# ViacheslavTimofeev/tpu_superresolution

Measured on AMD Instinct MI355X. Metric: HR pixels/sec, SwinIR x4 train step, 64x64 LR, bs=32/GPU, higher is better.
Workload: dtype bf16; 1 GPU; BASELINE cfg3: SwinIR classical x4 (dim 180, 6x6 blocks, window 8) train step = fwd + L1 + bwd + clip 1.0 + AdamW, 64x64 LR patches -> 256x256 HR, random-init weights, drop_path 0.1; every step starts from the seeded weights and fresh AdamW state; batch_per_gpu=32, global_batch=32, parallelism=dp1

## Files before the change

tpu_superresolution_amd/csrc/api.hip:

```cpp
#include <stdarg.h>
#include <stdio.h>
#include <string.h>

#include "adamw.h"
#include "kernels.h"
#include "wgrad.h"

static thread_local char g_err[512] = "";

SrkOptTls& srk_opt_tls() {
  static thread_local SrkOptTls t = {};
  return t;
}

static SrkOpt** opt_table() {
  static SrkOpt* table[SRK_NUM_OPTS] = {};
  return table;
}

void srk_opt_register(SrkOpt* o) {
  if (o->id >= 0 && o->id < SRK_NUM_OPTS) opt_table()[o->id] = o;
}

void srk_opt_scope_begin(SrkOptTls* saved) {
// ... 323 lines not shown
  srk_wgrad_stream_tune_get(&rows, &nt);
  return which == 0 ? rows : nt;
}

struct OptEntry {
  const char* name;
  int (*get)();
  int (*set)(int);
};

const OptEntry kOptions[] = {
    {"gemm_stream", [] { return srk_gemm_stream_enabled(); }, [](int v) { srk_gemm_stream_enable(v); return (int)SRK_OK; }},
    {"attn_bwd_fused", [] { return srk_attn_bwd_fused_enabled(); }, [](int v) { srk_attn_bwd_fused_enable(v); return (int)SRK_OK; }},
    {"attn_fused", [] { return srk_attn_fused_mode(); }, [](int v) { srk_attn_fused_enable(v); return (int)SRK_OK; }},
    {"wgrad_stream_w8", [] { return srk_wgrad_w8_enabled(); }, [](int v) { srk_wgrad_w8_enable(v); return (int)SRK_OK; }},
    {"block_light", [] { return srk_block_light_enabled(); }, [](int v) { srk_block_light_enable(v); return (int)SRK_OK; }},
    {"mlp_bwd_fused", [] { return srk_mlp_bwd_fused_enabled(); }, [](int v) { srk_mlp_bwd_fused_enable(v); return (int)SRK_OK; }},
    {"mlp_dgelu_store", [] { return srk_mlp_dgelu_store_enabled(); }, [](int v) { srk_mlp_dgelu_store_enable(v); return (int)SRK_OK; }},
    {"mlp_fused", [] { return srk_mlp_fused_enabled(); }, [](int v) { srk_mlp_fused_enable(v); return (int)SRK_OK; }},
    {"wgrad_stream", [] { return srk_wgrad_stream_enabled(); }, [](int v) { srk_wgrad_stream_enable(v); return (int)SRK_OK; }},
    {"conv_wgrad_taps", [] { return srk_conv_wgrad_taps_mode(); }, [](int v) { srk_conv_wgrad_taps_enable(v); return (int)SRK_OK; }},
    {"conv_wgrad_roll", [] { return srk_conv_wgrad_roll_enabled(); }, [](int v) { srk_conv_wgrad_roll_enable(v); return (int)SRK_OK; }},
    {"wgrad_partials", [] { return srk_wgrad_partials_enabled(); }, [](int v) { srk_wgrad_partials_enable(v); return (int)SRK_OK; }},
    {"wgrad_stream_rows", [] { return wtune_get(0); },
     [](int v) {
       SRK_REQUIRE(v == 32 || v == 64, SRK_E_SHAPE, "wgrad_stream_rows: 32/64");
       srk_wgrad_stream_tune(v, -1);
       return (int)SRK_OK;
     }},
    {"wgrad_stream_nt", [] { return wtune_get(1); }, [](int v) { srk_wgrad_stream_tune(0, v != 0); return (int)SRK_OK; }},
    {"gemm_stream_bm", [] { return tune_get(0); },
     [](int v) {
       SRK_REQUIRE(v == 0 || v == 16 || v == 32 || v == 64, SRK_E_SHAPE, "gemm_stream_bm: 0/16/32/64");
       return tune_set(0, v);
     }},
    {"gemm_stream_ks2", [] { return tune_get(1); }, [](int v) { return tune_set(1, v < 0 ? -1 : (v != 0)); }},
    {"gemm_stream_split", [] { return tune_get(2); }, [](int v) { return tune_set(2, v < 0 ? -1 : (v != 0)); }},
    {"gemm_stream_nb", [] { return tune_get(3); },
     [](int v) {
       SRK_REQUIRE(v == 0 || v == 4 || v == 8, SRK_E_SHAPE, "gemm_stream_nb: 0/4/8");
       return tune_set(3, v);
     }},
    {"probe_stride", [] { return g_probe.stride; },
     [](int v) {
       SRK_REQUIRE(v >= 1 && v <= 1024, SRK_E_SHAPE, "probe_stride: 1..1024");
       g_probe.stride = v;
// ... 246 lines not shown
```

tpu_superresolution_amd/csrc/common.h:

```cpp
#pragma once
#include <hip/hip_runtime.h>
#include <stdint.h>

#include "../../include/srk.h"

typedef unsigned short bf16_t;
typedef __attribute__((ext_vector_type(8))) short bf16x8_t;
typedef __attribute__((ext_vector_type(4))) short bf16x4_t;
typedef __attribute__((ext_vector_type(4))) float f32x4_t;

#define SRK_WAVE 64

void srk_set_error(const char* fmt, ...);
int srk_check_launch(const char* what);

constexpr int SRK_MAX_DEVICES = 64;
int srk_current_device();
int srk_device_cus();
enum SrkOptId {
  OPT_MLP_FUSED, OPT_MLP_BWD_FUSED, OPT_GEMM_STREAM, OPT_TUNE_BM, OPT_TUNE_KS2, OPT_TUNE_SPLIT, OPT_TUNE_NB, OPT_ATTN_BWD_FUSED,
  OPT_ATTN_FUSED, OPT_BLOCK_LIGHT, OPT_TAPS_ENABLED, OPT_TAPS_DMA, OPT_WGRAD_STREAM, OPT_WGRAD_ROWS, OPT_WGRAD_NT, OPT_WGRAD_W8,
  OPT_WGRAD_PARTIALS, OPT_MLP_DGELU_STORE, OPT_TAPS_ROLL, SRK_NUM_OPTS
};
struct SrkOptTls {
  int v[SRK_NUM_OPTS];
  unsigned on;
};
SrkOptTls& srk_opt_tls();
struct SrkOpt;
void srk_opt_register(SrkOpt* o);
void srk_opt_scope_begin(SrkOptTls* saved);
void srk_opt_scope_end(const SrkOptTls& saved);
struct SrkOpt {
  int id;
  int value;
  SrkOpt(int id_, int v) : id(id_), value(v) { srk_opt_register(this); }
  operator int() const {
    const SrkOptTls& t = srk_opt_tls();
    return ((t.on >> id) & 1u) ? t.v[id] : value;
  }
  SrkOpt& operator=(int v) {
    SrkOptTls& t = srk_opt_tls();
    if ((t.on >> id) & 1u) t.v[id] = v;
    else value = v;
    return *this;
// ... 224 lines not shown
```

tpu_superresolution_amd/csrc/gemm.hip:

```cpp
#include "gemm.h"
#include "gemm_rowep.h"

namespace {

constexpr int BM = 128;
constexpr int BK = 64;

#ifndef SRK_GEMM_DMA
#define SRK_GEMM_DMA 1
#endif
__device__ uint4 g_gemm_zero[1];

template <int LD>
struct RowCtx {
  long long base[4];
  int yx[4];
};

template <int LD, int EP, int NT, bool NARROW>
__global__ __launch_bounds__(256) void gemm_kernel(const GemmParams p) {
  constexpr int BN = NARROW ? 16 : NT * 32;
  constexpr int WPASS = NARROW ? 1 : BN / 32;
  extern __shared__ __attribute__((aligned(16))) unsigned char smem[];
  bf16_t* As = reinterpret_cast<bf16_t*>(smem);
// ... 336 lines not shown
  SRK_REQUIRE(p.A && p.Wt, SRK_E_NULL, "gemm: null operand");
  if (loader != LD_ROWS) {
    SRK_REQUIRE(p.CinP % 64 == 0 && p.K == 9 * p.CinP && p.M == p.B * p.H * p.W, SRK_E_SHAPE,
                "conv: inconsistent geometry K=%d CinP=%d M=%d B*H*W=%d", p.K, p.CinP, p.M, p.B * p.H * p.W);
    SRK_REQUIRE(p.H < 32768 && p.W < 32768, SRK_E_SHAPE, "conv: image too large");
    if (loader == LD_CONV3_PS) SRK_REQUIRE(p.Cs % 64 == 0 && p.CinP == p.r * p.r * p.Cs, SRK_E_SHAPE, "conv(ps-in): bad Cs");
  } else {
    SRK_REQUIRE(p.lda >= p.K && p.lda % 8 == 0, SRK_E_SHAPE, "gemm: bad lda %d", p.lda);
  }
  if (p.xn_out) {
    SRK_REQUIRE((epilogue == EP_PROJ_RES || epilogue == EP_RES) && (p.N == 64 || p.N == 128 || p.N == 192), SRK_E_SHAPE,
                "gemm: fused LayerNorm output needs a residual epilogue and N in {64,128,192} (N=%d)", p.N);
    SRK_REQUIRE(p.xn_mean && p.xn_rstd && p.xn_gamma && p.xn_beta, SRK_E_NULL, "gemm: fused LayerNorm: null pointer");
  }
  if (epilogue == EP_LNBWD) {
    SRK_REQUIRE(loader == LD_ROWS && (p.N == 64 || p.N == 128 || p.N == 192), SRK_E_SHAPE, "gemm(ln-bwd epilogue): N=%d must be one tile (64/128/192)", p.N);
    SRK_REQUIRE(p.ln_x && p.ln_mean && p.ln_rstd && p.ln_gamma && p.ln_dgamma && p.ln_dbeta && p.outf, SRK_E_NULL,
                "gemm(ln-bwd epilogue): null pointer");
  }
  if (loader == LD_ROWS) {
    const int rc = srk_launch_gemm_stream(epilogue, p, stream);
    if (rc != SRK_NOT_COVERED) return rc;
  }
#define CASE(LD, EP) \
  if (loader == LD && epilogue == EP) return dispatch_nt<LD, EP>(p, stream);
  CASE(LD_ROWS, EP_BF16)
  CASE(LD_ROWS, EP_QKV)
  CASE(LD_ROWS, EP_PROJ_RES)
  CASE(LD_ROWS, EP_GELU)
  CASE(LD_ROWS, EP_RES)
  CASE(LD_ROWS, EP_DGELU)
  CASE(LD_ROWS, EP_LNBWD)
  CASE(LD_ROWS, EP_LRELU)
  CASE(LD_ROWS, EP_DLRELU)
  CASE(LD_CONV3, EP_RES)
  CASE(LD_CONV3, EP_RES_BF16)
  CASE(LD_CONV3, EP_LRELU)
  CASE(LD_CONV3, EP_PS)
  CASE(LD_CONV3, EP_BF16)
  CASE(LD_CONV3, EP_DLRELU)
  CASE(LD_CONV3, EP_F32_BF16)
  CASE(LD_CONV3, EP_GELU)
  CASE(LD_CONV3, EP_DGELU)
  CASE(LD_ROWS, EP_RES_BF16)
  CASE(LD_CONV3_PS, EP_BF16)
  CASE(LD_CONV3_PS, EP_DLRELU)
// ... 7 lines not shown
```

tpu_superresolution_amd/csrc/gemm_stream.hip:

```cpp
#include <hip/hip_runtime.h>

#include "gemm.h"
#include "gemm_rowep.h"

namespace {

constexpr int SBN = 192;
constexpr int SBNP = SBN + 4;
constexpr int NC = SBN / 64;
constexpr int LDS_BUDGET = 160 * 1024;

#ifndef SRK_NT_GEMM
#define SRK_NT_GEMM 1
#endif
#ifndef SRK_NT_STORE_U
#define SRK_NT_STORE_U 1
#endif
typedef unsigned srk_u2 __attribute__((ext_vector_type(2)));
typedef float srk_f4 __attribute__((ext_vector_type(4)));
#ifndef SRK_NT_STORE_ALL
#define SRK_NT_STORE_ALL 0
#endif
__device__ __forceinline__ void st_u2(bf16_t* ptr, uint2 v) {
  if constexpr (SRK_NT_STORE_ALL != 0) __builtin_nontemporal_store(srk_u2{v.x, v.y}, reinterpret_cast<srk_u2*>(ptr));
  else *reinterpret_cast<uint2*>(ptr) = v;
}
// ... 365 lines not shown
      for (int c = 0; c < NC; ++c) {
        const float4 old = *reinterpret_cast<const float4*>(e0 + C::E32_BYTES + lr * (SBN * 4) + (64 * c + 4 * j16) * 4);
        float o[4] = {old.x, old.y, old.z, old.w};
        if (p.ln_skip) {
          const float4 sk = *reinterpret_cast<const float4*>(p.ln_skip + t_ * p.ldo + 64 * c + 4 * j16);
          o[0] += sk.x; o[1] += sk.y; o[2] += sk.z; o[3] += sk.w;
        }
#pragma unroll
        for (int e = 0; e < 4; ++e) {
          if (64 * c + 4 * j16 + e < p.ln_C) {
            o[e] += rstd * (dy[c][e] * gm[c][e] - s1 - xh[c][e] * s2);
            cg[c][e] += dy[c][e] * xh[c][e];
            cb[c][e] += dy[c][e];
          }
        }
        st_f4(dst + t_ * p.ldo + 64 * c + 4 * j16, make_float4(o[0], o[1], o[2], o[3]));
        if (p.outb)
          st_u2(p.outb + ro * p.ldo + 64 * c + 4 * j16, pack_bf4(o[0] * f, o[1] * f, o[2] * f, o[3] * f));
      }
    }
  }
}

template <int EP, int KC, int BM, bool KS2>
__global__ __launch_bounds__(512) void gemm_stream_kernel(const GemmParams p, int nchunk, int groups_per_xcd) {
  using C = StreamCfg<EP, KC, BM>;
  constexpr int K = C::K, R = C::R, MF = BM / 16;
  constexpr int KST = KS2 ? K / 64 : K / 32;
  extern __shared__ __attribute__((aligned(16))) unsigned char smem[];
  float* T = reinterpret_cast<float*>(smem);
  float* colred = reinterpret_cast<float*>(smem + C::T_BYTES);
  const unsigned smem_base = (unsigned)(size_t)smem;
  constexpr int SLOTS_OFF = C::T_BYTES + C::RED_BYTES;

  const int tid = threadIdx.x, lane = tid & 63;
  const int wave = __builtin_amdgcn_readfirstlane(tid >> 6);
  const int r16 = lane & 15, g = lane >> 4;

  const int xcd = blockIdx.x & 7, sx = blockIdx.x >> 3;
  const int chunk = sx % nchunk, gx = sx / nchunk;
  if (gx >= groups_per_xcd) return;
  const int n0 = chunk * SBN;
  const int Gm = 8 * groups_per_xcd, gi = gx * 8 + xcd;
  const int ntm = p.M / BM;
  const int nt = gi < ntm ? (ntm - gi + Gm - 1) / Gm : 0;
  if (nt == 0) return;

  const bool mfma_wave = KS2 || wave < 4;
  const int wn = wave & 3, kh = KS2 ? (wave >> 2) : 0;

  bf16x8_t wf[3][KST];
  if (mfma_wave) {
#pragma unroll
    for (int j = 0; j < 3; ++j)
#pragma unroll
      for (int s = 0; s < KST; ++s)
        wf[j][s] = *reinterpret_cast<const bf16x8_t*>(p.Wt + (long long)(n0 + wn * 48 + 16 * j + r16) * K + (kh * KST + s) * 32 + g * 8);
#pragma unroll
    for (int j = 0; j < 3; ++j)
#pragma unroll
      for (int s = 0; s < KST; ++s) asm volatile("" ::"v"(wf[j][s]));
  }
  if constexpr (EP == EP_LNBWD) {
// ... 657 lines not shown
    *state = -1;
    return SRK_OK;
  }
  if (hipFuncSetAttribute(fn, hipFuncAttributeMaxDynamicSharedMemorySize, lds) != hipSuccess) {
    srk_set_error("gemm(stream): cannot reserve %d bytes of LDS", lds);
    return SRK_E_LAUNCH;
  }
  *state = 1;
  return SRK_OK;
}

template <int EP, int KC, int BM, int NB>
int launch_split(const GemmParams& p, hipStream_t stream) {
  using S = SplitCfg<EP, KC, BM>;
  if constexpr (!S::VALID || BM % (4 * NB) != 0 || (NB == 8 && (KC > 3 || EP == EP_LNBWD))) {
    return SRK_NOT_COVERED;
  } else {
    static SrkPerDevice<int> configured_pd; int& configured = configured_pd.here();
    const int rc = stream_configure(&gemm_stream_split_kernel<EP, KC, BM, NB>, S::LDS, &configured);
    if (rc) return rc;
    if (configured < 0) return SRK_NOT_COVERED;
    const int nchunk = p.N / SBN;
    const int per_xcd = g_num_cus / 8;
    srk_probe_pre(FAM_GEMM_LINEAR, stream, p.flops, p.bytes);
    hipLaunchKernelGGL((gemm_stream_split_kernel<EP, KC, BM, NB>), dim3(per_xcd * 8), dim3(64 * (NB + 4)), S::LDS, stream, p, nchunk, per_xcd / nchunk);
    srk_probe_post(FAM_GEMM_LINEAR, stream);
    return srk_check_launch("gemm(stream-split)");
  }
}

template <int EP, int KC, int BM, bool KS2>
int launch_stream(const GemmParams& p, hipStream_t stream) {
  using C = StreamCfg<EP, KC, BM>;
  if constexpr (!C::VALID || (KC == 9 && !KS2)) {
    return SRK_NOT_COVERED;
  } else {
    static SrkPerDevice<int> configured_pd; int& configured = configured_pd.here();
    const int rcc = stream_configure(&gemm_stream_kernel<EP, KC, BM, KS2>, C::LDS, &configured);
    if (rcc) return rcc;
    if (configured < 0) return SRK_NOT_COVERED;
    const int nchunk = p.N / SBN;
    const int per_xcd = g_num_cus / 8;
    const int groups_per_xcd = per_xcd / nchunk;
    srk_probe_pre(FAM_GEMM_LINEAR, stream, p.flops, p.bytes);
    hipLaunchKernelGGL((gemm_stream_kernel<EP, KC, BM, KS2>), dim3(per_xcd * 8), dim3(512), C::LDS, stream, p, nchunk, groups_per_xcd);
    srk_probe_post(FAM_GEMM_LINEAR, stream);
    return srk_check_launch("gemm(stream)");
  }
}

template <int EP, int KC>
int launch_cfg(const GemmParams& p, hipStream_t stream, int bm, bool ks2) {
  if (bm == 16) return ks2 ? launch_stream<EP, KC, 16, true>(p, stream) : launch_stream<EP, KC, 16, false>(p, stream);
  if (bm == 32) return ks2 ? launch_stream<EP, KC, 32, true>(p, stream) : launch_stream<EP, KC, 32, false>(p, stream);
  if (bm == 64) return ks2 ? launch_stream<EP, KC, 64, true>(p, stream) : launch_stream<EP, KC, 64, false>(p, stream);
  return SRK_NOT_COVERED;
}

template <int EP, int KC>
int launch_split_bm(const GemmParams& p, hipStream_t stream, int bm, int nb) {
  if (nb == 8) {
    if (bm == 32) return launch_split<EP, KC, 32, 8>(p, stream);
    if (bm == 64) return launch_split<EP, KC, 64, 8>(p, stream);
    return SRK_NOT_COVERED;
  }
  if (bm == 16) return launch_split<EP, KC, 16, 4>(p, stream);
  if (bm == 32) return launch_split<EP, KC, 32, 4>(p, stream);
  if (bm == 64) return launch_split<EP, KC, 64, 4>(p, stream);
// ... 137 lines not shown
```

tpu_superresolution_amd/csrc/swinir.hip:

```cpp
#include <string.h>

#include <map>
#include <string>
#include <vector>

#include "kernels.h"
#include "wgrad.h"

namespace {

struct ParamEntry {
  std::string name;
  long long off, numel;
  int ndim;
  long long shape[4];
};

struct BlockW {
  long long n1w, n1b, rpb, qkvw, qkvb, projw, projb, n2w, n2b, fc1w, fc1b, fc2w, fc2b;
  long long Wqkv, WqkvT, Wproj, WprojT, Wfc1, Wfc1T, Wfc2, Wfc2T;
  long long bqkv, bproj, bfc1, bfc2, biasd;
  int nH, dh, CA, shift;
  float scale;
};
// ... 1233 lines not shown
        wq[2] = lin_wgrad(c, c.at<bf16_t>(w.gxbw), CP, c.at<bf16_t>(ba.ao), bw.CA, T, bw.Wproj, bw.bproj, fl_proj);
        int nslab;
        if (w.attn_recompute) {
          const int rc_abf = srk_launch_qkv_attn_bwd(c.at<bf16_t>(ba.xn1w), CP, c.packed + bw.Wqkv, c.side + bw.bqkv, bw.scale,
                                                     c.at<bf16_t>(w.gxbw), CP, c.packed + bw.WprojT, c.side + bw.biasd,
                                                     c.at<bf16_t>(w.dqkv), c.at<float>(w.slab), T / 64, bw.nH, bw.CA, CP, geom, st);
          SRK_REQUIRE(rc_abf != SRK_NOT_COVERED, SRK_E_STATE, "backward: the re-projecting attention backward cannot run but the "
                      "forward stored no q/k/v (option attn_bwd_fused changed between forward and backward?)");
          RUN(rc_abf);
          nslab = srk_qkv_attn_bwd_slabs(T / 64, bw.nH, bw.CA, CP);
        } else {
          {
            GemmParams g = {};
            g.A = c.at<bf16_t>(w.gxbw); g.lda = CP; g.Wt = c.packed + bw.WprojT; g.M = T; g.N = bw.CA; g.K = CP;
            g.outb = c.at<bf16_t>(w.dao); g.ldo = bw.CA; g.flops = fl_proj; g.bytes = (double)T * 4.0 * C + 2.0 * C * C;
            RUN(srk_launch_gemm(LD_ROWS, EP_BF16, g, st));
          }
          RUN(srk_launch_attn_bwd(c.at<bf16_t>(ba.qkv), c.side + bw.biasd, c.at<bf16_t>(w.dao), c.at<bf16_t>(w.dqkv),
                                  c.at<float>(w.slab), nullptr, T / 64, bw.nH, geom, bw.scale, st));
          nslab = srk_attn_bwd_slabs(T / 64, bw.nH, nullptr);
        }
        const RpbJob rpb = {c.at<float>(w.slab), grads + bw.rpb, nslab, bw.nH};
        wq[3] = lin_wgrad(c, c.at<bf16_t>(w.dqkv), 3 * bw.CA, c.at<bf16_t>(ba.xn1w), CP, T, bw.Wqkv, bw.bqkv, fl_qkv);
        RUN(srk_launch_wgrad_multi_rpb(wq, 4, &rpb, st));
        {
          GemmParams g = {};
          g.A = c.at<bf16_t>(w.dqkv); g.lda = 3 * bw.CA; g.Wt = c.packed + bw.WqkvT; g.M = T; g.N = CP; g.K = 3 * bw.CA;
          g.ldo = CP; g.flops = fl_qkv;
          g.bytes = (double)T * (6.0 * C + 4.0 * C + 8.0 * C + 2.0 * C) + 6.0 * C * C;
          if (fuse_ln) {
            g.outf = c.at<float>(w.gx2); g.outb = c.at<bf16_t>(j > 0 ? w.gxb2 : w.gxb); g.geom = geom; g.rowscale = j > 0 ? ds_prev_mlp : nullptr;
            g.rows_per_sample = HW;
            g.ln_skip = j > 0 ? nullptr : c.at<float>(w.gx);
            skip_folded = j == 0;
            g.ln_x = c.at<float>(ba.x_in); g.ln_mean = c.at<float>(ba.mean1); g.ln_rstd = c.at<float>(ba.rstd1);
            g.ln_gamma = params + bw.n1w; g.ln_dgamma = grads + bw.n1w; g.ln_dbeta = grads + bw.n1b; g.ln_C = C;
            g.ln_rows_window = 1; g.ln_stats_by_m = 1; g.ln_out_window = 0;
            RUN(srk_launch_gemm(LD_ROWS, EP_LNBWD, g, st));
          } else {
            g.outb = c.at<bf16_t>(w.dxn);
            RUN(srk_launch_gemm(LD_ROWS, EP_BF16, g, st));
            RUN(srk_launch_ln_bwd(c.at<bf16_t>(w.dxn), c.at<float>(ba.x_in), c.at<float>(ba.mean1), c.at<float>(ba.rstd1),
                                  params + bw.n1w, c.at<float>(w.gx2), c.at<bf16_t>(w.gxb2), grads + bw.n1w, grads + bw.n1b, T, C, CP,
                                  &geom, 1, 1, 0, 1, ds_prev_mlp, HW, st));
          }
        }
      }
      if (!skip_folded) RUN(srk_launch_add_f32_bf16(c.at<float>(w.gx), c.at<float>(w.gx2), c.at<bf16_t>(w.gxb), (long long)T * CP, st));
      RUN(unpack_group(c, l + 1, grads));
    } else {
      if (p->p_ape >= 0)
        RUN(srk_launch_ape_grad(c.at<float>(w.gx), grads + p->p_ape, B, p->cfg.img_size * p->cfg.img_size, C, CP, st));
      RUN(srk_launch_ln_bwd(c.at<bf16_t>(w.gxb), c.at<float>(w.f0), c.at<float>(w.mean_pe), c.at<float>(w.rstd_pe),
                            params + p->p_pe_w, c.at<float>(w.gx2), nullptr, grads + p->p_pe_w, grads + p->p_pe_b, T, C, CP, nullptr, 0,
                            0, 0, 0, nullptr, HW, st));
      RUN(srk_launch_add_bf16_into_f32(c.at<float>(w.gx2), c.at<bf16_t>(w.gfb), (long long)T * CP, st));
      RUN(srk_launch_stem_wgrad(c.at<float>(w.img4), c.at<float>(w.gx2), grads + p->p_conv_first_w, grads + p->p_conv_first_b, B, H, W,
                                p->Cimg, C, CP, st));
      RUN(unpack_group(c, 0, grads));
    }
  }
// ... 5 lines not shown
```

tpu_superresolution_amd/csrc/wgrad.h:

```cpp
#pragma once
#include "common.h"

struct WgradParams {
  const bf16_t* Y;
  int ldy;
  const bf16_t* X;
  int ldx;
  int M, N, K;
  float* dW;
  int ldw;
  float* db;
  int m_per;
  int conv;
  int B, H, W;
  double flops;
  double bytes;
  int r, Cs;
};

struct RpbJob {
  const float* slab;
  float* dtable;
  int nslab, nH;
};
// ... 12 lines not shown
__device__ __forceinline__ void rpb_reduce_block(const float* __restrict__ slab, float* __restrict__ dtable, int nslab, int nH, int i,
                                                 int h, float (*part)[64]) {
  const int lane = threadIdx.x & 63, wave = threadIdx.x >> 6;
  float a8[8] = {0.f, 0.f, 0.f, 0.f, 0.f, 0.f, 0.f, 0.f};
  const long long sstride = (long long)nH * 4096;
  const float* base = slab + ((long long)h * 64 + i) * 64 + lane;
  int sidx = wave;
  for (; sidx + 28 < nslab; sidx += 32) {
#pragma unroll
    for (int u = 0; u < 8; ++u) a8[u] += base[(sidx + 4 * u) * sstride];
  }
  for (; sidx < nslab; sidx += 4) a8[0] += base[sidx * sstride];
  part[wave][lane] = ((a8[0] + a8[1]) + (a8[2] + a8[3])) + ((a8[4] + a8[5]) + (a8[6] + a8[7]));
  __syncthreads();
  if (wave == 0) {
    const float v = part[0][lane] + part[1][lane] + part[2][lane] + part[3][lane];
    const int t = ((i >> 3) - (lane >> 3) + 7) * 15 + ((i & 7) - (lane & 7) + 7);
    atomicAdd(dtable + t * nH + h, v);
  }
}

constexpr int WS_SLAB_VEC = 9216;
constexpr size_t WS_WORKSPACE_BYTES = (size_t)256 * WS_SLAB_VEC * 16;
float* srk_wgrad_scratch(hipStream_t stream, size_t bytes);
void srk_wgrad_bind_workspace(void* ptr, size_t bytes, void** prev_ptr, size_t* prev_bytes);
void srk_wgrad_partials_enable(int on);
void srk_wgrad_w8_enable(int on);
void srk_wgrad_stream_tune(int rows, int nt);
int srk_wgrad_partials_enabled();
int srk_wgrad_stream_enabled();
int srk_wgrad_w8_enabled();
void srk_wgrad_stream_tune_get(int* rows, int* nt);

int srk_launch_wgrad(const WgradParams& p, hipStream_t stream);

#define SRK_WGRAD_NOT_COVERED 1
int srk_launch_conv_wgrad_taps(const WgradParams& p, hipStream_t stream);
void srk_conv_wgrad_taps_enable(int on);
int srk_conv_wgrad_taps_mode();
void srk_conv_wgrad_roll_enable(int on);
int srk_conv_wgrad_roll_enabled();
int srk_launch_smallconv_wgrad_mfma(const bf16_t* x, const float* gy, float* dW, float* db, int B, int H, int W, int Cin, int CinP, int Co,
                                    int CoP, hipStream_t stream);
int srk_launch_imghead_dgrad_mfma(const float* gy, const float* wgt, bf16_t* dx, int B, int H, int W, int Cin, int CinP, int Co, int CoP,
                                  hipStream_t stream);
void srk_wgrad_stream_enable(int on);
int srk_launch_wgrad_multi(const WgradParams* ps, int nprob, hipStream_t stream);
int srk_launch_wgrad_multi_rpb(const WgradParams* ps, int nprob, const RpbJob* rpb, hipStream_t stream);
int srk_launch_rpb_reduce(const float* slab, float* dtable, int nslab, int nH, hipStream_t stream);
```

tpu_superresolution_amd/csrc/wgrad.hip:

```cpp
#include "wgrad.h"

namespace {

template <int TA, int TB, bool CONV>
__global__ __launch_bounds__(256) void wgrad_kernel(const WgradMulti mp) {
  const int ntiles = mp.tile_begin[mp.nprob];
  const int logical = xcd_remap(blockIdx.x, gridDim.x);
  const int bsplit = logical / ntiles, btile = logical - bsplit * ntiles;
  int pi = 0;
  while (pi + 1 < mp.nprob && btile >= mp.tile_begin[pi + 1]) ++pi;
  const WgradParams& p = mp.p[pi];
  constexpr int TN = 64 * TA, TK = 64 * TB;
  constexpr int SY = TN + 16, SX = TK + 16;
  constexpr int PY = (64 * TN / 8) / 256;
  constexpr int PX = (64 * TK / 8) / 256;
  extern __shared__ __attribute__((aligned(16))) unsigned char smem[];
  bf16_t* Ys = reinterpret_cast<bf16_t*>(smem);
  bf16_t* Xs = Ys + 2 * 64 * SY;

  const int tid = threadIdx.x, lane = tid & 63, wave = tid >> 6;
  const int r16 = lane & 15, g = lane >> 4;
  const int wn = wave >> 1, wk = wave & 1;
  const int ntn = p.N / TN, ntk = p.K / TK;
  int bx = btile - mp.tile_begin[pi];
// ... 250 lines not shown
#pragma unroll
    for (int i = 0; i < FI; ++i)
#pragma unroll
      for (int j = 0; j < 6; ++j) slab[(size_t)(i * 6 + j) * mp.nsplit * 64] = acc[i][j];
  }
#pragma unroll
  for (int i = 0; i < FI; ++i) {
    const int n = n0 + wn * (16 * FI) + 16 * i + 4 * g;
    if (mp.partial == nullptr) {
#pragma unroll
      for (int j = 0; j < 6; ++j) {
        const int k = k0 + wk * 96 + 16 * j + r16;
#pragma unroll
        for (int e = 0; e < 4; ++e) atomicAdd(p.dW + (long long)(n + e) * p.ldw + k, acc[i][j][e]);
      }
    }
    if (do_bias && r16 == 0) {
#pragma unroll
      for (int e = 0; e < 4; ++e) atomicAdd(p.db + n + e, accb[i][e]);
    }
  }
}

__global__ __launch_bounds__(256) void wgrad_reduce_kernel(const WgradMulti mp) {
  if ((int)blockIdx.x >= 36 * mp.tile_begin[mp.nprob]) {
    __shared__ float part[4][64];
    const int b = blockIdx.x - 36 * mp.tile_begin[mp.nprob];
    rpb_reduce_block(mp.rpb.slab, mp.rpb.dtable, mp.rpb.nslab, mp.rpb.nH, b & 63, b >> 6, part);
    return;
  }
  const int btile = blockIdx.x / 36;
  const int q = (blockIdx.x - btile * 36) * 256 + threadIdx.x;
  int pi = 0;
  while (pi + 1 < mp.nprob && btile >= mp.tile_begin[pi + 1]) ++pi;
  const WgradParams& p = mp.p[pi];
  const int ntn = p.N / 192;
  const int bx = btile - mp.tile_begin[pi];
  const int tn = bx % ntn, tk = bx / ntn;
  const f32x4_t* src = reinterpret_cast<const f32x4_t*>(mp.partial) + ((size_t)btile * 144 + (q >> 6)) * mp.nsplit * 64 + (q & 63);
  f32x4_t sum = f32x4_t{0.f, 0.f, 0.f, 0.f};
  int s = 0;
  for (; s + 8 <= mp.nsplit; s += 8) {
    f32x4_t v[8];
#pragma unroll
    for (int u = 0; u < 8; ++u) v[u] = src[(s + u) * 64];
#pragma unroll
    for (int u = 0; u < 8; ++u) sum += v[u];
  }
  for (; s < mp.nsplit; ++s) sum += src[s * 64];
  const int lane = q & 63, t = q >> 6;
  const int fi = mp.w8 ? 3 : 6;
  const int j = t % 6, i = (t / 6) % fi, wave = t / (6 * fi);
  const int wn = wave >> 1, wk = wave & 1, r16 = lane & 15, g = lane >> 4;
  const int n = tn * 192 + wn * (16 * fi) + 16 * i + 4 * g;
  const int k = tk * 192 + wk * 96 + 16 * j + r16;
#pragma unroll
  for (int e = 0; e < 4; ++e) atomicAdd(p.dW + (long long)(n + e) * p.ldw + k, sum[e]);
}

thread_local const RpbJob* t_rpb = nullptr;
thread_local bool t_rpb_done = false;

SrkOpt g_wgrad_stream{OPT_WGRAD_STREAM, 1};
SrkOpt g_wgrad_rows{OPT_WGRAD_ROWS, 32};
SrkOpt g_wgrad_nt{OPT_WGRAD_NT, 1};
#ifndef SRK_WGRAD_W8_DEFAULT
#define SRK_WGRAD_W8_DEFAULT 1
#endif
SrkOpt g_wgrad_w8{OPT_WGRAD_W8, SRK_WGRAD_W8_DEFAULT};
SrkOpt g_wgrad_partials{OPT_WGRAD_PARTIALS, 1};

template <int TA, int TB, bool CONV>
int launch(const WgradParams* ps, int nprob, hipStream_t stream) {
  constexpr size_t lds = (size_t)2 * 64 * ((64 * TA + 16) + (64 * TB + 16)) * sizeof(bf16_t);
  static SrkPerDevice<bool> configured_pd; bool& configured = configured_pd.here();
  if (!configured) {
    if (hipFuncSetAttribute(reinterpret_cast<const void*>(&wgrad_kernel<TA, TB, CONV>),
                            hipFuncAttributeMaxDynamicSharedMemorySize, (int)lds) != hipSuccess) {
      srk_set_error("wgrad: cannot reserve %zu bytes of LDS", lds);
      return SRK_E_LAUNCH;
    }
    configured = true;
  }
  WgradMulti mp;
  mp.nprob = nprob;
  mp.partial = nullptr;
  mp.nsplit = 0;
  mp.rpb = RpbJob{nullptr, nullptr, 0, 0};
  mp.w8 = 0;
  int tiles = 0;
  double flops = 0.0, bytes = 0.0;
  for (int i = 0; i < nprob; ++i) {
    mp.p[i] = ps[i];
// ... 17 lines not shown
    if (ok) {
      constexpr int slds = WS_LDS_BYTES;
      using KernelFn = void (*)(const WgradMulti);
      static const KernelFn fns[8] = {&wgrad_stream_kernel<64, false, false>, &wgrad_stream_kernel<64, true, false>,
                                      &wgrad_stream_kernel<32, false, false>, &wgrad_stream_kernel<32, true, false>,
                                      &wgrad_stream_kernel<64, false, true>,  &wgrad_stream_kernel<64, true, true>,
                                      &wgrad_stream_kernel<32, false, true>,  &wgrad_stream_kernel<32, true, true>};
      static SrkPerDevice<bool> sconf_pd; bool& sconf = sconf_pd.here();
      if (!sconf) {
        for (KernelFn f : fns)
          if (hipFuncSetAttribute(reinterpret_cast<const void*>(f), hipFuncAttributeMaxDynamicSharedMemorySize, slds) != hipSuccess) {
            srk_set_error("wgrad(stream): cannot reserve %d bytes of LDS", slds);
            return SRK_E_LAUNCH;
          }
        sconf = true;
      }
      const KernelFn fn = fns[(g_wgrad_w8 ? 4 : 0) + (g_wgrad_rows == 32 ? 2 : 0) + (g_wgrad_nt ? 1 : 0)];
      mp.nsplit = splits;
      mp.w8 = g_wgrad_w8;
      mp.partial = g_wgrad_partials && splits > 1 ? srk_wgrad_scratch(stream, (size_t)tiles * splits * WS_SLAB_VEC * 16) : nullptr;
      srk_probe_pre(fam, stream, flops, bytes);
      hipLaunchKernelGGL(fn, dim3(tiles * splits), dim3(g_wgrad_w8 ? 512 : 256), slds, stream, mp);
      if (mp.partial) {
        int extra = 0;
        if (t_rpb && t_rpb->slab) {
          mp.rpb = *t_rpb;
          extra = 64 * t_rpb->nH;
          t_rpb_done = true;
        }
        hipLaunchKernelGGL(wgrad_reduce_kernel, dim3(tiles * 36 + extra), dim3(256), 0, stream, mp);
      }
      srk_probe_post(fam, stream);
      return srk_check_launch("wgrad(stream)");
    }
  }
  srk_probe_pre(fam, stream, flops, bytes);
  hipLaunchKernelGGL((wgrad_kernel<TA, TB, CONV>), dim3(tiles * splits), dim3(256), lds, stream, mp);
  srk_probe_post(fam, stream);
  return srk_check_launch("wgrad");
}

inline void tile_class(const WgradParams& p, int& a, int& b) {
  a = p.N % 192 == 0 ? 3 : (p.N % 128 == 0 ? 2 : 1);
  b = p.K % 192 == 0 ? 3 : (p.K % 128 == 0 ? 2 : 1);
}

template <bool CONV>
int dispatch(const WgradParams* ps, int nprob, hipStream_t stream) {
  int a, b;
  tile_class(ps[0], a, b);
#define WCASE(A, B) \
  if (a == A && b == B) return launch<A, B, CONV>(ps, nprob, stream);
  WCASE(3, 3) WCASE(3, 1) WCASE(1, 3) WCASE(2, 2) WCASE(2, 1) WCASE(1, 2) WCASE(1, 1) WCASE(3, 2) WCASE(2, 3)
// ... 2 lines not shown
  return SRK_E_UNSUPPORTED;
}

int validate(const WgradParams& p) {
  SRK_REQUIRE(p.M > 0 && p.N % 64 == 0 && p.K % 64 == 0, SRK_E_SHAPE, "wgrad: bad M/N/K %d/%d/%d", p.M, p.N, p.K);
  SRK_REQUIRE(p.Y && p.X && p.dW, SRK_E_NULL, "wgrad: null operand");
  if (p.conv) {
    SRK_REQUIRE(p.M == p.B * p.H * p.W, SRK_E_SHAPE, "wgrad(conv): M != B*H*W");
    if (p.r > 1) SRK_REQUIRE(p.Cs % 8 == 0 && p.N == p.r * p.r * p.Cs, SRK_E_SHAPE, "wgrad(conv,ps): bad Cs");
  }
  return SRK_OK;
}

}

void srk_wgrad_stream_enable(int on) { g_wgrad_stream = on ? 1 : 0; }
void srk_wgrad_partials_enable(int on) { g_wgrad_partials = on ? 1 : 0; }
void srk_wgrad_w8_enable(int on) { g_wgrad_w8 = on ? 1 : 0; }
void srk_wgrad_stream_tune(int rows, int nt) {
  if (rows == 32 || rows == 64) g_wgrad_rows = rows;
  if (nt >= 0) g_wgrad_nt = nt ? 1 : 0;
}
int srk_wgrad_partials_enabled() { return g_wgrad_partials; }
int srk_wgrad_stream_enabled() { return g_wgrad_stream; }
int srk_wgrad_w8_enabled() { return g_wgrad_w8; }
void srk_wgrad_stream_tune_get(int* rows, int* nt) { *rows = g_wgrad_rows; *nt = g_wgrad_nt; }

namespace {
thread_local float* t_wgrad_ws = nullptr;
thread_local size_t t_wgrad_ws_bytes = 0;
}
void srk_wgrad_bind_workspace(void* ptr, size_t bytes, void** prev_ptr, size_t* prev_bytes) {
  if (prev_ptr) *prev_ptr = t_wgrad_ws;
  if (prev_bytes) *prev_bytes = t_wgrad_ws_bytes;
  t_wgrad_ws = static_cast<float*>(ptr);
  t_wgrad_ws_bytes = ptr ? bytes : 0;
}
float* srk_wgrad_scratch(hipStream_t, size_t bytes) { return bytes <= t_wgrad_ws_bytes ? t_wgrad_ws : nullptr; }

int srk_launch_wgrad(const WgradParams& p, hipStream_t stream) {
  int rc = validate(p);
  if (rc) return rc;
  if (p.conv) {
    rc = srk_launch_conv_wgrad_taps(p, stream);
    if (rc != SRK_WGRAD_NOT_COVERED) return rc;
  }
  return p.conv ? dispatch<true>(&p, 1, stream) : dispatch<false>(&p, 1, stream);
}

int srk_launch_wgrad_multi_rpb(const WgradParams* ps, int nprob, const RpbJob* rpb, hipStream_t stream) {
  t_rpb = rpb;
  t_rpb_done = false;
  int rc = srk_launch_wgrad_multi(ps, nprob, stream);
  t_rpb = nullptr;
  if (rc == SRK_OK && rpb && rpb->slab && !t_rpb_done) rc = srk_launch_rpb_reduce(rpb->slab, rpb->dtable, rpb->nslab, rpb->nH, stream);
  return rc;
}

int srk_launch_wgrad_multi(const WgradParams* ps, int nprob, hipStream_t stream) {
  SRK_REQUIRE(nprob >= 1 && nprob <= 4, SRK_E_SHAPE, "wgrad_multi: nprob=%d", nprob);
  bool same = true;
  int a0, b0;
  tile_class(ps[0], a0, b0);
  for (int i = 0; i < nprob; ++i) {
    int rc = validate(ps[i]);
    if (rc) return rc;
    int a, b;
    tile_class(ps[i], a, b);
    same = same && a == a0 && b == b0 && ps[i].M == ps[0].M && !ps[i].conv;
  }
  if (same) return dispatch<false>(ps, nprob, stream);
  for (int i = 0; i < nprob; ++i) {
    int rc = srk_launch_wgrad(ps[i], stream);
    if (rc) return rc;
  }
  return SRK_OK;
}
```

Baseline: 76.56 million HR pixels/s.

## Fold wgrad split-K reduction into the following LN-backward dgrad stream GEMM

The split-K partial reduction (plus the relative-position-bias table reduction) that followed the attention wgrad launch is now deferred and handed to the next EP_LNBWD stream GEMM. There, the first four waves of every block do a share of the reduction before the GEMM work begins. This removes a separate reduce kernel launch and lets the reduction use blocks that would otherwise sit idle or wait. In exchange, the GEMM prologue gets longer, register pressure in that kernel may rise, and a fallback flush is needed on paths that do not take the job.

Result: no change. 77.08 million HR pixels/s, median of 6 (+0.7%).

```diff
diff --git a/tpu_superresolution_amd/csrc/api.hip b/tpu_superresolution_amd/csrc/api.hip
--- a/tpu_superresolution_amd/csrc/api.hip
+++ b/tpu_superresolution_amd/csrc/api.hip
@@ -369,6 +369,13 @@
     {"conv_wgrad_taps", [] { return srk_conv_wgrad_taps_mode(); }, [](int v) { srk_conv_wgrad_taps_enable(v); return (int)SRK_OK; }},
     {"conv_wgrad_roll", [] { return srk_conv_wgrad_roll_enabled(); }, [](int v) { srk_conv_wgrad_roll_enable(v); return (int)SRK_OK; }},
     {"wgrad_partials", [] { return srk_wgrad_partials_enabled(); }, [](int v) { srk_wgrad_partials_enable(v); return (int)SRK_OK; }},
+    {"wgrad_reduce_ride", [] { return srk_wgrad_reduce_ride_enabled(); }, [](int v) { srk_wgrad_reduce_ride_enable(v); return (int)SRK_OK; }},
+    {"wgrad_reduce_ridden", [] { return srk_wgrad_reduce_ridden(); },
+     [](int v) {
+       SRK_REQUIRE(v == 0, SRK_E_SHAPE, "wgrad_reduce_ridden: read-only (0 clears it)");
+       srk_wgrad_reduce_ridden_clear();
+       return (int)SRK_OK;
+     }},
     {"wgrad_stream_rows", [] { return wtune_get(0); },
      [](int v) {
        SRK_REQUIRE(v == 32 || v == 64, SRK_E_SHAPE, "wgrad_stream_rows: 32/64");
diff --git a/tpu_superresolution_amd/csrc/common.h b/tpu_superresolution_amd/csrc/common.h
--- a/tpu_superresolution_amd/csrc/common.h
+++ b/tpu_superresolution_amd/csrc/common.h
@@ -20,7 +20,7 @@
 enum SrkOptId {
   OPT_MLP_FUSED, OPT_MLP_BWD_FUSED, OPT_GEMM_STREAM, OPT_TUNE_BM, OPT_TUNE_KS2, OPT_TUNE_SPLIT, OPT_TUNE_NB, OPT_ATTN_BWD_FUSED,
   OPT_ATTN_FUSED, OPT_BLOCK_LIGHT, OPT_TAPS_ENABLED, OPT_TAPS_DMA, OPT_WGRAD_STREAM, OPT_WGRAD_ROWS, OPT_WGRAD_NT, OPT_WGRAD_W8,
-  OPT_WGRAD_PARTIALS, OPT_MLP_DGELU_STORE, OPT_TAPS_ROLL, SRK_NUM_OPTS
+  OPT_WGRAD_PARTIALS, OPT_MLP_DGELU_STORE, OPT_TAPS_ROLL, OPT_WGRAD_RIDE, SRK_NUM_OPTS
 };
 struct SrkOptTls {
   int v[SRK_NUM_OPTS];
diff --git a/tpu_superresolution_amd/csrc/gemm.hip b/tpu_superresolution_amd/csrc/gemm.hip
--- a/tpu_superresolution_amd/csrc/gemm.hip
+++ b/tpu_superresolution_amd/csrc/gemm.hip
@@ -1,5 +1,6 @@
 #include "gemm.h"
 #include "gemm_rowep.h"
+#include "wgrad.h"
 
 namespace {
 
@@ -382,6 +383,10 @@
     const int rc = srk_launch_gemm_stream(epilogue, p, stream);
     if (rc != SRK_NOT_COVERED) return rc;
   }
+  if (epilogue == EP_LNBWD) {
+    const int rcf = srk_wgrad_ride_flush(stream);
+    if (rcf) return rcf;
+  }
 #define CASE(LD, EP) \
   if (loader == LD && epilogue == EP) return dispatch_nt<LD, EP>(p, stream);
   CASE(LD_ROWS, EP_BF16)
diff --git a/tpu_superresolution_amd/csrc/gemm_stream.hip b/tpu_superresolution_amd/csrc/gemm_stream.hip
--- a/tpu_superresolution_amd/csrc/gemm_stream.hip
+++ b/tpu_superresolution_amd/csrc/gemm_stream.hip
@@ -2,6 +2,9 @@
 
 #include "gemm.h"
 #include "gemm_rowep.h"
+#include "wgrad.h"
+
+#include <type_traits>
 
 namespace {
 
@@ -413,8 +416,12 @@
   }
 }
 
+struct NoRide {};
+template <int EP>
+using RideArg = std::conditional_t<EP == EP_LNBWD, WgradReduceJob, NoRide>;
+
 template <int EP, int KC, int BM, bool KS2>
-__global__ __launch_bounds__(512) void gemm_stream_kernel(const GemmParams p, int nchunk, int groups_per_xcd) {
+__global__ __launch_bounds__(512) void gemm_stream_kernel(const GemmParams p, int nchunk, int groups_per_xcd, const RideArg<EP> ride) {
   using C = StreamCfg<EP, KC, BM>;
   constexpr int K = C::K, R = C::R, MF = BM / 16;
   constexpr int KST = KS2 ? K / 64 : K / 32;
@@ -430,6 +437,11 @@
 
   const int xcd = blockIdx.x & 7, sx = blockIdx.x >> 3;
   const int chunk = sx % nchunk, gx = sx / nchunk;
+  if constexpr (EP == EP_LNBWD) {
+    if (ride.partial != nullptr && wave < 4) wgrad_reduce_share(ride, blockIdx.x, gridDim.x, tid);
+    asm volatile("" ::: "memory");
+    __builtin_amdgcn_sched_barrier(0);
+  }
   if (gx >= groups_per_xcd) return;
   const int n0 = chunk * SBN;
   const int Gm = 8 * groups_per_xcd, gi = gx * 8 + xcd;
@@ -1133,6 +1145,10 @@
     if (configured < 0) return SRK_NOT_COVERED;
     const int nchunk = p.N / SBN;
     const int per_xcd = g_num_cus / 8;
+    if constexpr (EP == EP_LNBWD) {
+      const int rcf = srk_wgrad_ride_flush(stream);
+      if (rcf) return rcf;
+    }
     srk_probe_pre(FAM_GEMM_LINEAR, stream, p.flops, p.bytes);
     hipLaunchKernelGGL((gemm_stream_split_kernel<EP, KC, BM, NB>), dim3(per_xcd * 8), dim3(64 * (NB + 4)), S::LDS, stream, p, nchunk, per_xcd / nchunk);
     srk_probe_post(FAM_GEMM_LINEAR, stream);
@@ -1153,8 +1169,10 @@
     const int nchunk = p.N / SBN;
     const int per_xcd = g_num_cus / 8;
     const int groups_per_xcd = per_xcd / nchunk;
+    RideArg<EP> ride = {};
+    if constexpr (EP == EP_LNBWD) srk_wgrad_ride_take(&ride);
     srk_probe_pre(FAM_GEMM_LINEAR, stream, p.flops, p.bytes);
-    hipLaunchKernelGGL((gemm_stream_kernel<EP, KC, BM, KS2>), dim3(per_xcd * 8), dim3(512), C::LDS, stream, p, nchunk, groups_per_xcd);
+    hipLaunchKernelGGL((gemm_stream_kernel<EP, KC, BM, KS2>), dim3(per_xcd * 8), dim3(512), C::LDS, stream, p, nchunk, groups_per_xcd, ride);
     srk_probe_post(FAM_GEMM_LINEAR, stream);
     return srk_check_launch("gemm(stream)");
   }
diff --git a/tpu_superresolution_amd/csrc/swinir.hip b/tpu_superresolution_amd/csrc/swinir.hip
--- a/tpu_superresolution_amd/csrc/swinir.hip
+++ b/tpu_superresolution_amd/csrc/swinir.hip
@@ -1279,7 +1279,10 @@
         }
         const RpbJob rpb = {c.at<float>(w.slab), grads + bw.rpb, nslab, bw.nH};
         wq[3] = lin_wgrad(c, c.at<bf16_t>(w.dqkv), 3 * bw.CA, c.at<bf16_t>(ba.xn1w), CP, T, bw.Wqkv, bw.bqkv, fl_qkv);
-        RUN(srk_launch_wgrad_multi_rpb(wq, 4, &rpb, st));
+        WgradReduceJob rjob = {};
+        const bool ride = fuse_ln && srk_wgrad_reduce_ride_enabled();
+        RUN(srk_launch_wgrad_multi_rpb(wq, 4, &rpb, st, ride ? &rjob : nullptr));
+        if (rjob.partial) srk_wgrad_ride_offer(rjob);
         {
           GemmParams g = {};
           g.A = c.at<bf16_t>(w.dqkv); g.lda = 3 * bw.CA; g.Wt = c.packed + bw.WqkvT; g.M = T; g.N = CP; g.K = 3 * bw.CA;
@@ -1293,7 +1296,10 @@
             g.ln_x = c.at<float>(ba.x_in); g.ln_mean = c.at<float>(ba.mean1); g.ln_rstd = c.at<float>(ba.rstd1);
             g.ln_gamma = params + bw.n1w; g.ln_dgamma = grads + bw.n1w; g.ln_dbeta = grads + bw.n1b; g.ln_C = C;
             g.ln_rows_window = 1; g.ln_stats_by_m = 1; g.ln_out_window = 0;
-            RUN(srk_launch_gemm(LD_ROWS, EP_LNBWD, g, st));
+            const int rc_dgrad = srk_launch_gemm(LD_ROWS, EP_LNBWD, g, st);
+            const int rc_flush = srk_wgrad_ride_flush(st);
+            RUN(rc_dgrad);
+            RUN(rc_flush);
           } else {
             g.outb = c.at<bf16_t>(w.dxn);
             RUN(srk_launch_gemm(LD_ROWS, EP_BF16, g, st));
diff --git a/tpu_superresolution_amd/csrc/wgrad.h b/tpu_superresolution_amd/csrc/wgrad.h
--- a/tpu_superresolution_amd/csrc/wgrad.h
+++ b/tpu_superresolution_amd/csrc/wgrad.h
@@ -58,6 +58,123 @@
 
 constexpr int WS_SLAB_VEC = 9216;
 constexpr size_t WS_WORKSPACE_BYTES = (size_t)256 * WS_SLAB_VEC * 16;
+
+__device__ __forceinline__ void rpb_reduce_wave(const float* __restrict__ slab, float* __restrict__ dtable, int nslab, int nH, int i,
+                                                int h, int lane) {
+  float a[4][8];
+#pragma unroll
+  for (int w = 0; w < 4; ++w)
+#pragma unroll
+    for (int u = 0; u < 8; ++u) a[w][u] = 0.f;
+  const long long sstride = (long long)nH * 4096;
+  const float* base = slab + ((long long)h * 64 + i) * 64 + lane;
+  int s0 = 0;
+  for (; s0 + 63 < nslab; s0 += 64) {
+    float t[2][4][8];
+#pragma unroll
+    for (int k = 0; k < 2; ++k)
+#pragma unroll
+      for (int w = 0; w < 4; ++w)
+#pragma unroll
+        for (int u = 0; u < 8; ++u) t[k][w][u] = base[(s0 + 32 * k + w + 4 * u) * sstride];
+    __builtin_amdgcn_sched_barrier(0);
+#pragma unroll
+    for (int k = 0; k < 2; ++k)
+#pragma unroll
+      for (int w = 0; w < 4; ++w)
+#pragma unroll
+        for (int u = 0; u < 8; ++u) a[w][u] += t[k][w][u];
+  }
+  for (; s0 + 31 < nslab; s0 += 32) {
+    float t[4][8];
+#pragma unroll
+    for (int w = 0; w < 4; ++w)
+#pragma unroll
+      for (int u = 0; u < 8; ++u) t[w][u] = base[(s0 + w + 4 * u) * sstride];
+    __builtin_amdgcn_sched_barrier(0);
+#pragma unroll
+    for (int w = 0; w < 4; ++w)
+#pragma unroll
+      for (int u = 0; u < 8; ++u) a[w][u] += t[w][u];
+  }
+  float v = 0.f;
+#pragma unroll
+  for (int w = 0; w < 4; ++w) {
+    int sidx = s0 + w;
+    for (; sidx + 28 < nslab; sidx += 32) {
+#pragma unroll
+      for (int u = 0; u < 8; ++u) a[w][u] += base[(sidx + 4 * u) * sstride];
+    }
+    for (; sidx < nslab; sidx += 4) a[w][0] += base[sidx * sstride];
+    const float pw = ((a[w][0] + a[w][1]) + (a[w][2] + a[w][3])) + ((a[w][4] + a[w][5]) + (a[w][6] + a[w][7]));
+    v = w == 0 ? pw : v + pw;
+  }
+  const int t = ((i >> 3) - (lane >> 3) + 7) * 15 + ((i & 7) - (lane & 7) + 7);
+  atomicAdd(dtable + t * nH + h, v);
+}
+
+struct WgradReduceProb {
+  float* dW;
+  int ldw;
+  int ntn;
+  int tile_begin;
+};
+struct WgradReduceJob {
+  const float* partial;
+  int nsplit, w8, ntiles, nprob;
+  WgradReduceProb p[4];
+  RpbJob rpb;
+};
+
+template <int NB>
+__device__ __forceinline__ void wgrad_reduce_batch(const f32x4_t* __restrict__ src, f32x4_t& sum) {
+  f32x4_t v[NB];
+#pragma unroll
+  for (int u = 0; u < NB; ++u) v[u] = src[u * 64];
+  __builtin_amdgcn_sched_barrier(0);
+#pragma unroll
+  for (int u = 0; u < NB; ++u) sum += v[u];
+}
+
+__device__ __forceinline__ void wgrad_reduce_vector(const WgradReduceJob& jb, int vec) {
+  const int btile = vec / WS_SLAB_VEC, q = vec - btile * WS_SLAB_VEC;
+  float* dW = jb.p[0].dW;
+  int ldw = jb.p[0].ldw, ntn = jb.p[0].ntn, tb = 0;
+#pragma unroll
+  for (int i = 1; i < 4; ++i)
+    if (i < jb.nprob && btile >= jb.p[i].tile_begin) {
+      dW = jb.p[i].dW; ldw = jb.p[i].ldw; ntn = jb.p[i].ntn; tb = jb.p[i].tile_begin;
+    }
+  const int bx = btile - tb;
+  const int tk = bx / ntn, tn = bx - tk * ntn;
+  const f32x4_t* src = reinterpret_cast<const f32x4_t*>(jb.partial) + ((size_t)btile * 144 + (q >> 6)) * jb.nsplit * 64 + (q & 63);
+  f32x4_t sum = f32x4_t{0.f, 0.f, 0.f, 0.f};
+  int s = 0;
+  for (; s + 32 <= jb.nsplit; s += 32) wgrad_reduce_batch<32>(src + s * 64, sum);
+  for (; s + 8 <= jb.nsplit; s += 8) wgrad_reduce_batch<8>(src + s * 64, sum);
+  for (; s < jb.nsplit; ++s) sum += src[s * 64];
+  const int lane = q & 63, t = q >> 6;
+  const int fi = jb.w8 ? 3 : 6;
+  const int j = t % 6, i = (t / 6) % fi, wave = t / (6 * fi);
+  const int wn = wave >> 1, wk = wave & 1, r16 = lane & 15, g = lane >> 4;
+  const int n = tn * 192 + wn * (16 * fi) + 16 * i + 4 * g;
+  const int k = tk * 192 + wk * 96 + 16 * j + r16;
+#pragma unroll
+  for (int e = 0; e < 4; ++e) atomicAdd(dW + (long long)(n + e) * ldw + k, sum[e]);
+}
+
+__device__ __forceinline__ void wgrad_reduce_share(const WgradReduceJob& jb, int b, int G, int t) {
+  const unsigned total = (unsigned)jb.ntiles * WS_SLAB_VEC;
+  const int v0 = (int)(total * (unsigned)b / (unsigned)G), v1 = (int)(total * (unsigned)(b + 1) / (unsigned)G);
+  for (int v = v0 + t; v < v1; v += 256) wgrad_reduce_vector(jb, v);
+  if (jb.rpb.slab != nullptr) {
+    const int U = 64 * jb.rpb.nH;
+    const int u0 = U * b / G, u1 = U * (b + 1) / G;
+    for (int u = u0 + 3 - (t >> 6); u < u1; u += 4)
+      rpb_reduce_wave(jb.rpb.slab, jb.rpb.dtable, jb.rpb.nslab, jb.rpb.nH, u & 63, u >> 6, t & 63);
+  }
+}
+
 float* srk_wgrad_scratch(hipStream_t stream, size_t bytes);
 void srk_wgrad_bind_workspace(void* ptr, size_t bytes, void** prev_ptr, size_t* prev_bytes);
 void srk_wgrad_partials_enable(int on);
@@ -82,5 +199,13 @@
                                   hipStream_t stream);
 void srk_wgrad_stream_enable(int on);
 int srk_launch_wgrad_multi(const WgradParams* ps, int nprob, hipStream_t stream);
-int srk_launch_wgrad_multi_rpb(const WgradParams* ps, int nprob, const RpbJob* rpb, hipStream_t stream);
+int srk_launch_wgrad_multi_rpb(const WgradParams* ps, int nprob, const RpbJob* rpb, hipStream_t stream, WgradReduceJob* defer = nullptr);
+int srk_launch_wgrad_reduce(const WgradReduceJob& job, hipStream_t stream);
+void srk_wgrad_ride_offer(const WgradReduceJob& job);
+bool srk_wgrad_ride_take(WgradReduceJob* out);
+int srk_wgrad_ride_flush(hipStream_t stream);
+void srk_wgrad_reduce_ride_enable(int on);
+int srk_wgrad_reduce_ride_enabled();
+int srk_wgrad_reduce_ridden();
+void srk_wgrad_reduce_ridden_clear();
 int srk_launch_rpb_reduce(const float* slab, float* dtable, int nslab, int nH, hipStream_t stream);
diff --git a/tpu_superresolution_amd/csrc/wgrad.hip b/tpu_superresolution_amd/csrc/wgrad.hip
--- a/tpu_superresolution_amd/csrc/wgrad.hip
+++ b/tpu_superresolution_amd/csrc/wgrad.hip
@@ -1,4 +1,6 @@
 #include "wgrad.h"
+
+#include <atomic>
 
 namespace {
 
@@ -296,44 +298,27 @@
   }
 }
 
-__global__ __launch_bounds__(256) void wgrad_reduce_kernel(const WgradMulti mp) {
-  if ((int)blockIdx.x >= 36 * mp.tile_begin[mp.nprob]) {
+__global__ __launch_bounds__(256) void wgrad_reduce_kernel(const WgradReduceJob jb) {
+  if ((int)blockIdx.x >= 36 * jb.ntiles) {
     __shared__ float part[4][64];
-    const int b = blockIdx.x - 36 * mp.tile_begin[mp.nprob];
-    rpb_reduce_block(mp.rpb.slab, mp.rpb.dtable, mp.rpb.nslab, mp.rpb.nH, b & 63, b >> 6, part);
+    const int b = blockIdx.x - 36 * jb.ntiles;
+    rpb_reduce_block(jb.rpb.slab, jb.rpb.dtable, jb.rpb.nslab, jb.rpb.nH, b & 63, b >> 6, part);
     return;
   }
-  const int btile = blockIdx.x / 36;
-  const int q = (blockIdx.x - btile * 36) * 256 + threadIdx.x;
-  int pi = 0;
-  while (pi + 1 < mp.nprob && btile >= mp.tile_begin[pi + 1]) ++pi;
-  const WgradParams& p = mp.p[pi];
-  const int ntn = p.N / 192;
-  const int bx = btile - mp.tile_begin[pi];
-  const int tn = bx % ntn, tk = bx / ntn;
-  const f32x4_t* src = reinterpret_cast<const f32x4_t*>(mp.partial) + ((size_t)btile * 144 + (q >> 6)) * mp.nsplit * 64 + (q & 63);
-  f32x4_t sum = f32x4_t{0.f, 0.f, 0.f, 0.f};
-  int s = 0;
-  for (; s + 8 <= mp.nsplit; s += 8) {
-    f32x4_t v[8];
-#pragma unroll
-    for (int u = 0; u < 8; ++u) v[u] = src[(s + u) * 64];
-#pragma unroll
-    for (int u = 0; u < 8; ++u) sum += v[u];
-  }
-  for (; s < mp.nsplit; ++s) sum += src[s * 64];
-  const int lane = q & 63, t = q >> 6;
-  const int fi = mp.w8 ? 3 : 6;
-  const int j = t % 6, i = (t / 6) % fi, wave = t / (6 * fi);
-  const int wn = wave >> 1, wk = wave & 1, r16 = lane & 15, g = lane >> 4;
-  const int n = tn * 192 + wn * (16 * fi) + 16 * i + 4 * g;
-  const int k = tk * 192 + wk * 96 + 16 * j + r16;
-#pragma unroll
-  for (int e = 0; e < 4; ++e) atomicAdd(p.dW + (long long)(n + e) * p.ldw + k, sum[e]);
+  wgrad_reduce_vector(jb, blockIdx.x * 256 + threadIdx.x);
 }
 
 thread_local const RpbJob* t_rpb = nullptr;
 thread_local bool t_rpb_done = false;
+thread_local WgradReduceJob* t_defer = nullptr;
+thread_local WgradReduceJob t_ride = {};
+std::atomic<int> g_ridden{0};
+
+int launch_reduce(const WgradReduceJob& jb, hipStream_t stream) {
+  const int extra = jb.rpb.slab ? 64 * jb.rpb.nH : 0;
+  hipLaunchKernelGGL(wgrad_reduce_kernel, dim3(jb.ntiles * 36 + extra), dim3(256), 0, stream, jb);
+  return srk_check_launch("wgrad(reduce)");
+}
 
 SrkOpt g_wgrad_stream{OPT_WGRAD_STREAM, 1};
 SrkOpt g_wgrad_rows{OPT_WGRAD_ROWS, 32};
@@ -343,6 +328,7 @@
 #endif
 SrkOpt g_wgrad_w8{OPT_WGRAD_W8, SRK_WGRAD_W8_DEFAULT};
 SrkOpt g_wgrad_partials{OPT_WGRAD_PARTIALS, 1};
+SrkOpt g_wgrad_ride{OPT_WGRAD_RIDE, 1};
 
 template <int TA, int TB, bool CONV>
 int launch(const WgradParams* ps, int nprob, hipStream_t stream) {
@@ -406,13 +392,18 @@
       srk_probe_pre(fam, stream, flops, bytes);
       hipLaunchKernelGGL(fn, dim3(tiles * splits), dim3(g_wgrad_w8 ? 512 : 256), slds, stream, mp);
       if (mp.partial) {
-        int extra = 0;
+        WgradReduceJob jb = {};
+        jb.partial = mp.partial; jb.nsplit = splits; jb.w8 = mp.w8; jb.ntiles = tiles; jb.nprob = nprob;
+        for (int i = 0; i < nprob; ++i) jb.p[i] = WgradReduceProb{ps[i].dW, ps[i].ldw, ps[i].N / 192, mp.tile_begin[i]};
         if (t_rpb && t_rpb->slab) {
-          mp.rpb = *t_rpb;
-          extra = 64 * t_rpb->nH;
+          jb.rpb = *t_rpb;
           t_rpb_done = true;
         }
-        hipLaunchKernelGGL(wgrad_reduce_kernel, dim3(tiles * 36 + extra), dim3(256), 0, stream, mp);
+        if (t_defer) {
+          *t_defer = jb;
+        } else {
+          hipLaunchKernelGGL(wgrad_reduce_kernel, dim3(tiles * 36 + (jb.rpb.slab ? 64 * jb.rpb.nH : 0)), dim3(256), 0, stream, jb);
+        }
       }
       srk_probe_post(fam, stream);
       return srk_check_launch("wgrad(stream)");
@@ -461,6 +452,29 @@
   if (nt >= 0) g_wgrad_nt = nt ? 1 : 0;
 }
 int srk_wgrad_partials_enabled() { return g_wgrad_partials; }
+void srk_wgrad_reduce_ride_enable(int on) { g_wgrad_ride = on ? 1 : 0; }
+int srk_wgrad_reduce_ride_enabled() { return g_wgrad_ride; }
+int srk_wgrad_reduce_ridden() { return g_ridden.load(); }
+void srk_wgrad_reduce_ridden_clear() { g_ridden.store(0); }
+
+int srk_launch_wgrad_reduce(const WgradReduceJob& job, hipStream_t stream) {
+  if (!job.partial) return SRK_OK;
+  return launch_reduce(job, stream);
+}
+void srk_wgrad_ride_offer(const WgradReduceJob& job) { t_ride = job; }
+bool srk_wgrad_ride_take(WgradReduceJob* out) {
+  if (!t_ride.partial) return false;
+  *out = t_ride;
+  t_ride.partial = nullptr;
+  g_ridden.fetch_add(1);
+  return true;
+}
+int srk_wgrad_ride_flush(hipStream_t stream) {
+  if (!t_ride.partial) return SRK_OK;
+  const WgradReduceJob jb = t_ride;
+  t_ride.partial = nullptr;
+  return launch_reduce(jb, stream);
+}
 int srk_wgrad_stream_enabled() { return g_wgrad_stream; }
 int srk_wgrad_w8_enabled() { return g_wgrad_w8; }
 void srk_wgrad_stream_tune_get(int* rows, int* nt) { *rows = g_wgrad_rows; *nt = g_wgrad_nt; }
@@ -487,11 +501,14 @@
   return p.conv ? dispatch<true>(&p, 1, stream) : dispatch<false>(&p, 1, stream);
 }
 
-int srk_launch_wgrad_multi_rpb(const WgradParams* ps, int nprob, const RpbJob* rpb, hipStream_t stream) {
+int srk_launch_wgrad_multi_rpb(const WgradParams* ps, int nprob, const RpbJob* rpb, hipStream_t stream, WgradReduceJob* defer) {
   t_rpb = rpb;
   t_rpb_done = false;
+  if (defer) *defer = WgradReduceJob{};
+  t_defer = defer;
   int rc = srk_launch_wgrad_multi(ps, nprob, stream);
   t_rpb = nullptr;
+  t_defer = nullptr;
   if (rc == SRK_OK && rpb && rpb->slab && !t_rpb_done) rc = srk_launch_rpb_reduce(rpb->slab, rpb->dtable, rpb->nslab, rpb->nH, stream);
   return rc;
 }
@@ -509,6 +526,7 @@
     same = same && a == a0 && b == b0 && ps[i].M == ps[0].M && !ps[i].conv;
   }
   if (same) return dispatch<false>(ps, nprob, stream);
+  t_defer = nullptr;
   for (int i = 0; i < nprob; ++i) {
     int rc = srk_launch_wgrad(ps[i], stream);
     if (rc) return rc;
```
